# montyhall/bot7

Measured on AMD Instinct MI355X. Metric: EI candidates scored/sec at N=2048,d=32, higher is better.
Workload: dtype f64

## Files before the change

### bot7_amd/build.py

```python
import concurrent.futures
import os
import subprocess
import sys

HERE = os.path.dirname(os.path.abspath(__file__))
ROOT = os.path.dirname(HERE)
CSRC = os.path.join(HERE, "csrc")
BUILD = os.path.join(HERE, "_build")
OUT = os.path.join(HERE, "libbot7hip.so")
SOURCES = ["context.hip", "grid_api.hip", "gp_api.hip", "nominate.hip", "blr_api.hip", "sobol.hip", "covar.hip", "potrf.hip", "potrf_persist.hip", "posterior.hip", "score.hip", "extras.hip", "comm.hip", "group.hip", "blr_small.hip", "gp_small.hip", "kpost_small.hip", "batch.hip", "mes.hip"]
DIAG_ONLY_SOURCES = ["nll_small.hip"]
DIAG_OUT = os.path.join(ROOT, "tools", "_build", "libbot7hip_diag.so")
HEADERS = [os.path.join(CSRC, "b7_internal.h"), os.path.join(CSRC, "gemm_f64.h"), os.path.join(CSRC, "potrf_diag.h"), os.path.join(CSRC, "comm_rccl.h"), os.path.join(CSRC, "ksx_exp.h"), os.path.join(CSRC, "exp_table.h"), os.path.join(CSRC, "mes_math.h"),
           os.path.join(ROOT, "include", "bot7hip.h")]
HIPCC = os.environ.get("HIPCC", "/opt/rocm/bin/hipcc")
FLAGS = ["-O3", "-std=c++17", "-fPIC", "--offload-arch=gfx950", "-fno-fast-math", "-Wall",
         "-I" + os.path.join(ROOT, "include"), "-I" + CSRC, "-I/opt/rocm/include"]


def _stale(target, deps):
    if not os.path.exists(target):
        return True
    t = os.path.getmtime(target)
    return any(os.path.getmtime(d) > t for d in deps)


EXTRA_FLAGS = {"covar.hip": ["-mllvm", "-amdgpu-mfma-vgpr-form"], "batch.hip": ["-mllvm", "-amdgpu-mfma-vgpr-form"]}


def _compile(src, diag=False):
    obj = os.path.join(BUILD, ("diag_" if diag else "") + src.replace(".hip", ".o"))
    path = os.path.join(CSRC, src)
    if _stale(obj, [path] + HEADERS + [os.path.abspath(__file__)]):
        subprocess.check_call([HIPCC] + FLAGS + EXTRA_FLAGS.get(src, []) + (["-DB7_DIAG"] if diag else []) + ["-c", path, "-o", obj])
        return obj, True
    return obj, False


def _mentions_diag(src):
    return "B7_DIAG" in open(os.path.join(CSRC, src)).read()


def build_diag(verbose=False):
    build()
    os.makedirs(os.path.dirname(DIAG_OUT), exist_ok=True)
    todo = [s for s in SOURCES if _mentions_diag(s)] + DIAG_ONLY_SOURCES
    with concurrent.futures.ThreadPoolExecutor(max_workers=min(8, len(todo))) as ex:
        res = dict(zip(todo, ex.map(lambda s: _compile(s, True), todo)))
    objs = [res[s][0] if s in res else os.path.join(BUILD, s.replace(".hip", ".o")) for s in SOURCES + DIAG_ONLY_SOURCES]
    if any(ch for _, ch in res.values()) or _stale(DIAG_OUT, objs):
        subprocess.check_call([HIPCC, "-shared", "-fPIC", "--offload-arch=gfx950", "-o", DIAG_OUT] + objs +
                              ["-ldl", "-Wl,-rpath,/opt/rocm/lib", "-Wl,--no-undefined", "-Wl,-Bsymbolic"])
        if verbose:
            print("built", DIAG_OUT)
    return DIAG_OUT


def posterior_isa():
    out = os.path.join(BUILD, "posterior.s")
    path = os.path.join(CSRC, "posterior.hip")
    if _stale(out, [path] + HEADERS + [os.path.abspath(__file__)]):
        subprocess.check_call([HIPCC] + [f for f in FLAGS if f != "-fPIC"] + ["-S", "--cuda-device-only", "-Wno-unused-command-line-argument",
                                                                            path, "-o", out])
# ... 72 lines not shown
```

### bot7_amd/csrc/b7_internal.h

```cpp
#pragma once
#include <hip/hip_runtime.h>
#include <stddef.h>
#include <stdint.h>

#include <map>
#include <string>
#include <vector>

#include "bot7hip.h"

constexpr int B7_NPAD = 128;
constexpr int B7_PANEL = 64;
constexpr int B7_PERSIST_NMAX = 4096;
constexpr int B7_MROWS = 256;
constexpr int B7_MAX_D = 96;

constexpr int B7_TAB_VAL = 0;
constexpr int B7_TAB_IDX = 1;
constexpr int B7_TAB_STATUS = 2;
constexpr int B7_TAB_ROWS = 3;
constexpr int B7_TAB_ROW0 = 4;
constexpr int B7_TAB_W = B7_TAB_ROW0 + B7_MAX_D;
constexpr int B7_MAX_WORLD = 64;

// ... 89 lines not shown
  DevBuf w;
  DevBuf zsc;
  DevBuf zss;
  DevBuf K;
  DevBuf L;
  DevBuf Linv;
  DevBuf W;
  DevBuf dinv;
  DevBuf alpha;
  DevBuf resid;
  DevBuf atmp;
  DevBuf info;
  DevBuf ybuf;

  bool predicted = false;
  int64_t Mpred = 0;
  DevBuf mu;
  DevBuf var;
  DevBuf acc;
  bool acc_valid = false;
  int spin_us = 500;
  bool npad_small = true;
  bool potrf_small = true;
  bool blr_small = true;
  double fmin_scalar = 0.0;
  bool acc_fresh = false;
  int acc_kind = 0;
  DevBuf ks;
  size_t ks_bytes = (size_t)4 << 30;
  int diag_variant = 1;
  int inverse_inline = 1;
  PinnedBlock *pinned = nullptr, *pinned_dev = nullptr;
  std::vector<double> net_host;
  PinBuf pin_blr;
  PinBuf pin_eval;
  PinBuf pin_nll;
  bool fmin_staged = false;
  bool potrf_attrs_set = false;
  bool linv_done = false;
  int potrf_sched = 3;
  int syrk_small = 1;
  int potrf_defer = 1;
  int potrf_group = 2;
  struct JobList { DevBuf buf; int n = 0; };
  std::map<int, JobList> pjobs_cache;
  DevBuf pstamps;
  int pjobs_nb = 0, pjobs_n = 0;
  DevBuf bhyp, bw, bzsc, bzss, bK, bL, bdinv, bflags, binfo, bresid, bterms, bLinv, balpha, bmu, bvar;
  bool persist_attr_set = false, persist_stamps = false;
  int persist_helpers = 0;
  int persist_aborts = 0;
  int nll_small = 1;
  bool kpost_small = true;
  bool fit_small = true;
  int persist_fault = -1;
  int potrf_sched_saved = 0;
  DevBuf part;
  DevBuf ystar, mes_ticket;
  DevBuf mes_user;
  int mes_levels = 8;
  int mes_S = 0, mes_K = 0, mes_nb = 0;
  int64_t mes_M = 0;
  int mes_slot = 0;
  bool mes_valid = false;
  DevBuf ticket;
  DevBuf scratch;
  DevBuf tmpgrid;
  DevBuf tmpmu, tmpvar;
  DevBuf fant;
  DevBuf bel;
  DevBuf belvec;
  PinBuf pin_bel;
  DevBuf feat;
  size_t feat_zeroed_bytes = 0;
  int feat_z = -1;
  int64_t Mfeat = 0;
  int zdim = 0;
  uint64_t feat_version = 0, grid_version = 0;
  DevBuf netbuf;

  void *comm = nullptr;
  int comm_rank = 0, comm_world = 1;
  DevBuf slots;
  uint64_t *tab_host = nullptr;
  uint64_t *tab_host_dev = nullptr;
  struct b7_group *group = nullptr;
  bool group_busy = false;
  bool win_valid = false;
  int64_t win_idx1 = 0;
  int win_rank = -1, win_d = 0;
  double win_row[B7_MAX_D];
  int64_t shard_rows[B7_MAX_WORLD];
  int shard_world = 0;

  hipEvent_t tev[B7_MAX_TIMERS][2];
  bool tev_init = false;
  bool profile = false;
  std::map<std::string, PhaseStat> phases;
  struct PendingPhase { const char *name; hipEvent_t e0, e1; };
  std::vector<PendingPhase> pending;
  std::vector<hipEvent_t> free_events;
  hipEvent_t phase_e0 = nullptr;
};

int b7_fail(b7_ctx *c, int code, const char *fmt, ...);
#define B7_HIP(c, expr)                                                                          \
// ... 38 lines not shown
  int64_t s_w = 0, s_zsc = 0, s_zsh = 0, s_out = 0;
  const double *amp = nullptr;
  int64_t s_alpha = 0, s_mu = 0;
  const double *mean = nullptr;
};
struct ObsSet {
  const double *zsc;
  const double *zsh;
  int npad;
  const double *w = nullptr;
  KBatchDesc batch;
};
int launch_prep_obs_aux(b7_ctx *c, const double *xobs, const double *ls_dev, int N, int npad, double *zsc,
                        double *zsh);
int launch_k_generic(b7_ctx *c, const double *xq, int64_t rows, int64_t Mtotal, const ObsSet &o, double *out);
int launch_prep_obs(b7_ctx *c, const double *xobs, const double *lenscale_sq_dev, int N, int d);
int launch_kxx(b7_ctx *c, double diag_add);
int launch_ksx_batch(b7_ctx *c, int S, const double *xq, int64_t rows, int64_t Mtotal, const double *w, const double *zsc,
                     const double *zss, const double *amp_dev, const double *mean_dev, const double *alpha, double *ks,
                     int64_t s_out, double *mu, int64_t s_mu);
int launch_kxx_batch(b7_ctx *c, int B, const double *ls_dev, const double *amp_dev, const double *noise_dev, double *w,
                     double *zsc, double *zss, double *K);
int launch_ksx(b7_ctx *c, const double *xq, int64_t row0, int64_t rows, int64_t Mtotal, int d, double *ks,
               double *mu, int ycols);

struct FactorNote {
  bool alpha_done = false;
  int *report_written = nullptr;
};
int launch_potrf(b7_ctx *c, double extra, bool with_inverse, int *report_hint = nullptr, FactorNote *note = nullptr);
int launch_trtri(b7_ctx *c);
int launch_potrf_persist(b7_ctx *c, double extra, bool with_inverse);
int launch_nll_batch(b7_ctx *c, int B, const double *K, double *L, double *dinv, unsigned *flags, int *info,
                     const double *resid, double *terms);
int launch_nll_one(b7_ctx *c, const double *K, double *L, double *dinv, unsigned *flags, int *info, const double *resid,
                   double *terms, double extra);
size_t persist_flag_words_host(int nb);
int launch_potrf_small(b7_ctx *c, int B, const double *K, double *L, double *Linv, double *dinv, const double *resid, double *alpha,
                       double extra, int *info, int *report_dev, int64_t sK, int64_t sL, int64_t sdinv, int64_t svec, int sinfo);
int launch_blr_head_small(b7_ctx *c, const double *Z, int N, int z, int ldz, const double *yv, double alpha_prec, double beta,
                          int *report_dev);
int launch_blr_heads_small(b7_ctx *c, int S, const double *Z, int N, int z, int ldz, const double *yraw_dev, const double *hyp3_dev,
                           double *L, double *Linv, double *m, double *b, int *info, int *report_dev, double *terms);
int launch_post_heads(b7_ctx *c, int S, const double *Linv, const double *feat, int64_t rows, int64_t Mtotal, double *var, int64_t svar,
                      const double *zero_dev, const double *invbeta_dev);
int launch_gemv_rows_batch(b7_ctx *c, int S, const double *A, int lda, const double *x, int64_t sx, int n, const double *base_dev,
                           int64_t rows, double *y, int64_t sy);
int launch_nll_small(b7_ctx *c, int B, const double *hyp_dev, const double *hyp_host, double *terms_dev, int *info_dev,
                     unsigned *done_dev);
bool kpost_small_applies(const b7_ctx *c);
int launch_kpost_small(b7_ctx *c, int S, const double *xq, int64_t M, const double *w, const double *zsc, const double *zss,
                       const double *Linv, const double *alpha, const double *hyp_dev, double amp, double noise, double mean,
                       double *mu, double *var, int64_t sout);
bool gp_small_applies(const b7_ctx *c);
static inline bool fit_small_applies(const b7_ctx *c) {
  return c->fit_small && c->potrf_sched == 3 && c->inverse_inline && gp_small_applies(c);
}
int launch_nll_small8(b7_ctx *c, int B, const double *hyp_dev, const double *hyp_host, double *terms_dev, int *info_dev,
                      unsigned *done_dev);
int launch_fit_small(b7_ctx *c, int B, const double *hyp_dev, const double *hyp_host, double *hyp_out, double *w, double *zsc,
                     double *zss, double *L, double *Linv, double *dinv, double *alpha, double *resid, int *info_dev,
                     int *report_dev);
int launch_alpha(b7_ctx *c, int *report_dev = nullptr, int report_words = 0, const FactorNote &note = FactorNote());
int launch_alpha_batch(b7_ctx *c, int B, const double *Linv, const double *resid, double *alpha, const int *report_src = nullptr,
                       int *report_dev = nullptr, int report_words = 0);
int launch_fit_batch(b7_ctx *c, int B, const double *K, double *L, double *Linv, double *dinv, unsigned *flags, int *info);
int launch_nll_terms(b7_ctx *c, double *out_dev);
int launch_fro_norm_sq(b7_ctx *c, const double *A, int n, int ld, double *out_dev);
int launch_set_identity(b7_ctx *c);

int launch_post(b7_ctx *c, const double *ks, int64_t row0, int64_t rows, int64_t Mtotal, double *var);
int launch_post_batch(b7_ctx *c, int S, const double *Linv, const double *ks, int64_t sks, int64_t rows, int64_t Mtotal,
                      double *var, int64_t svar, const double *amp_dev, const double *noise_dev);

int launch_mean_multi(b7_ctx *c, const double *ks, int64_t row0, int64_t rows, int64_t Mtotal, double *mu);
int launch_gemm_nt(b7_ctx *c, const double *A, int lda, const double *B, int ldb, double *C, int ldc, int m, int n,
                   int k);
int launch_fantasy_cov(b7_ctx *c, const double *kpp, const double *g, double *S, int P, double diag_add);
int launch_fantasy_factor(b7_ctx *c, double *S, double *dinv_tmp, int *info_dev);
int launch_fantasy_sample(b7_ctx *c, const double *Lp, const double *mu, int P, int n, uint64_t seed, double *out);
int launch_add_diag(b7_ctx *c, double *S, int ld, int n, double v);

int launch_append_finalize(b7_ctx *c, const double *krow, const double *lvec, const double *uvec, const double *evec,
                           int *status_dev);
int launch_append_vectors(b7_ctx *c, const double *krow, double *lvec, double *uvec, double *part, double *evec);
int launch_mlp_forward(b7_ctx *c, const double *X, int64_t M, int d, const double *net_dev, const int *dims,
                       int n_layers, int activation, double *out, int ld_out);
int launch_mlp_forward_mean(b7_ctx *c, const double *X, int64_t M, int d, const double *net_dev, const int *dims,
                            int n_layers, int activation, double *out, int ld_out, const double *mvec, double mean0,
                            double *mu, bool *mean_done);
int launch_gemv_rows(b7_ctx *c, const double *A, int lda, const double *x, int n, double base, int64_t row0,
                     int64_t rows, int64_t Mtotal, double *y);
int launch_transpose_pad(b7_ctx *c, const double *Z, int n, int ldz, int z, double *Zt, int zpad, int nk);
int launch_blr_assemble(b7_ctx *c, const double *G, double *K, int z, int zpad, double alpha_prec, double beta);

int launch_score(b7_ctx *c, ScoreParams p, const double *mu, const double *var, int64_t M, int ycols, double *out, bool accumulate);
int launch_score_batch(b7_ctx *c, const ScoreParams &p, double *acc, int64_t M);
int launch_finish(b7_ctx *c, double *acc, int64_t M, double divisor, double *best_val, int64_t *best_idx1, bool logacc = false);
int launch_fill(b7_ctx *c, double *p, int64_t n, double v);
int launch_finish_slot(b7_ctx *c, double *acc, int64_t M, double divisor, uint64_t *tab_dev, int rank, int world,
                       int64_t offset, const double *grid, int d, bool all_slots, uint64_t *host_rec = nullptr,
                       unsigned *host_done = nullptr, bool logacc = false);

struct ExclRows {
  int n = 0;
  long long row[B7_BATCH_MAX];
// ... 105 lines not shown
```

### bot7_amd/csrc/context.hip

```cpp
#include <stdarg.h>
#include <stdio.h>
#include <stdlib.h>
#include <string.h>

#include "b7_internal.h"

static thread_local std::string g_create_err;

int b7_fail(b7_ctx *c, int code, const char *fmt, ...) {
  char buf[512];
  va_list ap;
  va_start(ap, fmt);
  vsnprintf(buf, sizeof(buf), fmt, ap);
  va_end(ap);
  if (c)
    c->err = buf;
  else
    g_create_err = buf;
  return code;
}

int b7_ensure(b7_ctx *c, DevBuf &b, size_t bytes) {
  if (bytes == 0) bytes = 16;
  if (b.cap >= bytes) return B7_OK;
// ... 73 lines not shown
int npad_of(const b7_ctx *c, int64_t n) { return (c->npad_small && n <= 64) ? 64 : (int)round_up(n, B7_NPAD); }

static int timers_init(b7_ctx *c) {
  if (c->tev_init) return B7_OK;
  for (int i = 0; i < B7_MAX_TIMERS; ++i) {
    B7_HIP(c, hipEventCreate(&c->tev[i][0]));
    B7_HIP(c, hipEventCreate(&c->tev[i][1]));
  }
  c->tev_init = true;
  return B7_OK;
}

extern "C" {

int b7_abi_version(void) { return B7_ABI_VERSION; }

int b7_create(b7_ctx **out, int device_id) {
  if (!out) return b7_fail(nullptr, B7_ERR_INVALID, "b7_create: out is NULL");
  *out = nullptr;
  int ndev = 0;
  hipError_t e = hipGetDeviceCount(&ndev);
  if (e != hipSuccess || ndev <= 0)
    return b7_fail(nullptr, B7_ERR_HIP, "no HIP device available (%s); libbot7hip has no CPU path",
                   e == hipSuccess ? "device count 0" : hipGetErrorString(e));
  if (device_id < 0 || device_id >= ndev)
    return b7_fail(nullptr, B7_ERR_INVALID, "device_id %d out of range [0,%d)", device_id, ndev);
  e = hipSetDevice(device_id);
  if (e != hipSuccess) return b7_fail(nullptr, B7_ERR_HIP, "hipSetDevice: %s", hipGetErrorString(e));
  hipDeviceProp_t prop;
  e = hipGetDeviceProperties(&prop, device_id);
  if (e != hipSuccess) return b7_fail(nullptr, B7_ERR_HIP, "hipGetDeviceProperties: %s", hipGetErrorString(e));
  if (strncmp(prop.gcnArchName, "gfx950", 6) != 0)
    return b7_fail(nullptr, B7_ERR_UNSUPPORTED, "device %d is %s; libbot7hip is built for gfx950 only", device_id,
                   prop.gcnArchName);
  b7_ctx *c = new b7_ctx();
  c->device = device_id;
  c->cus = prop.multiProcessorCount;
  b7_gp_default_opts(&c->opts);
  if (const char *pv = getenv("B7_SPIN_US")) c->spin_us = atoi(pv);
#ifdef B7_DIAG
  if (const char *pv = getenv("B7_DIAG_VARIANT")) c->diag_variant = atoi(pv);
  if (const char *pv = getenv("B7_NPAD_SMALL")) c->npad_small = atoi(pv) != 0;
  if (const char *pv = getenv("B7_POTRF_SMALL")) c->potrf_small = atoi(pv) != 0;
  if (getenv("B7_POTRF_SCHED") || getenv("B7_DIAG_VARIANT") || getenv("B7_INVERSE_INLINE")) c->potrf_small = c->fit_small = false;
  if (const char *pv = getenv("B7_BLR_SMALL")) c->blr_small = atoi(pv) != 0;
  if (const char *pv = getenv("B7_INVERSE_INLINE")) c->inverse_inline = atoi(pv);
  if (const char *pv = getenv("B7_POTRF_SCHED")) c->potrf_sched = atoi(pv);
  c->persist_stamps = getenv("B7_PERSIST_STAMPS") != nullptr;
  if (const char *pv = getenv("B7_PERSIST_HELPERS")) c->persist_helpers = atoi(pv);
  if (const char *pv = getenv("B7_PERSIST_FAULT")) c->persist_fault = atoi(pv);
  if (const char *pv = getenv("B7_NLL_SMALL")) c->nll_small = atoi(pv);
  if (const char *pv = getenv("B7_FIT_SMALL")) c->fit_small = atoi(pv) != 0;
  if (const char *pv = getenv("B7_KPOST_SMALL")) c->kpost_small = atoi(pv) != 0;
  if (const char *pv = getenv("B7_SYRK_SMALL")) c->syrk_small = atoi(pv) ? 1 : 0;
  if (const char *pv = getenv("B7_POTRF_DEFER")) c->potrf_defer = atoi(pv) ? 1 : 0;
  if (const char *pv = getenv("B7_POTRF_GROUP")) {
    const int g = atoi(pv);
    if (g >= 1 && g <= 8) c->potrf_group = g;
  }
#endif
  e = hipStreamCreateWithFlags(&c->stream, hipStreamNonBlocking);
  if (e == hipSuccess) e = hipEventCreateWithFlags(&c->ev_fit, hipEventDisableTiming);
  if (e == hipSuccess) e = hipHostMalloc((void **)&c->pinned, B7_PINNED_BYTES, hipHostMallocMapped);
  if (e == hipSuccess) e = hipHostGetDevicePointer((void **)&c->pinned_dev, c->pinned, 0);
  if (e != hipSuccess) {
    if (c->pinned) (void)hipHostFree(c->pinned);
    if (c->stream) (void)hipStreamDestroy(c->stream);
    delete c;
    return b7_fail(nullptr, B7_ERR_HIP, "stream / pinned result block creation: %s", hipGetErrorString(e));
  }
  if (b7_ensure(c, c->scratch, B7_SCRATCH_BYTES) != B7_OK) {
    g_create_err = c->err;
    b7_destroy(c);
    return B7_ERR_NOMEM;
  }
  *out = c;
  return B7_OK;
}

void b7_destroy(b7_ctx *c) {
  if (!c) return;
  (void)hipSetDevice(c->device);
  (void)hipStreamSynchronize(c->stream);
  (void)b7_comm_destroy(c);
  DevBuf *all[] = {&c->grid[0], &c->grid[1], &c->xobs, &c->w,     &c->zsc,  &c->zss,     &c->K,      &c->L,
                   &c->Linv,    &c->W,       &c->dinv, &c->alpha, &c->resid, &c->info,   &c->ybuf,   &c->mu,
                   &c->var,     &c->acc,     &c->ks,   &c->part,  &c->scratch, &c->tmpgrid, &c->tmpmu, &c->tmpvar, &c->fant, &c->feat, &c->netbuf, &c->atmp, &c->slots, &c->pstamps,
                   &c->bhyp, &c->bw, &c->bzsc, &c->bzss, &c->bK, &c->bL, &c->bdinv, &c->bflags, &c->binfo, &c->bresid, &c->bterms,
                   &c->bLinv, &c->balpha, &c->bmu, &c->bvar, &c->ticket, &c->bel, &c->belvec, &c->ystar, &c->mes_ticket, &c->mes_user};
  for (auto &kv : c->pjobs_cache) b7_release(kv.second.buf);
  for (DevBuf *b : all) b7_release(*b);
  if (c->tev_init)
    for (int i = 0; i < B7_MAX_TIMERS; ++i) {
      (void)hipEventDestroy(c->tev[i][0]);
      (void)hipEventDestroy(c->tev[i][1]);
    }
  resolve_phases(c);
  if (c->pinned) (void)hipHostFree(c->pinned);
  for (PinBuf *b : {&c->pin_eval, &c->pin_blr, &c->pin_nll, &c->pin_bel})
    if (b->host) (void)hipHostFree(b->host);
  if (c->tab_host) (void)hipHostFree(c->tab_host);
  for (hipEvent_t e : c->free_events) (void)hipEventDestroy(e);
  if (c->phase_e0) (void)hipEventDestroy(c->phase_e0);
  if (c->ev_fit) (void)hipEventDestroy(c->ev_fit);
  (void)hipStreamDestroy(c->stream);
  delete c;
// ... 72 lines not shown
```

### bot7_amd/csrc/gp_api.hip

```cpp
#include <math.h>
#include <string.h>

#include <chrono>

#include "b7_internal.h"

extern "C" __global__ void __launch_bounds__(256) resid_kernel(const double *__restrict__ y, double *__restrict__ r, int64_t nreal,
                                                               int64_t ntotal, double mean) {
  const int64_t e = (int64_t)blockIdx.x * blockDim.x + threadIdx.x;
  if (e < ntotal) r[e] = e < nreal ? y[e] - mean : 0.0;
}

extern "C" __global__ void __launch_bounds__(256) resid_batch_kernel(const double *__restrict__ y, double *__restrict__ r, int N,
                                                                     int Npad, const double *__restrict__ mean) {
  const int i = blockIdx.x * blockDim.x + threadIdx.x, b = blockIdx.y;
  if (i < Npad) r[(int64_t)b * Npad + i] = i < N ? y[i] - mean[b] : 0.0;
}

void launch_resid_batch(b7_ctx *c, int B, const double *mean_dev) {
  hipLaunchKernelGGL(resid_batch_kernel, dim3((c->Npad + 255) / 256, B), dim3(256), 0, c->stream, (const double *)c->ybuf.p,
                     (double *)c->bresid.p, c->N, c->Npad, mean_dev);
}

void persist_gave_up(b7_ctx *c) {
// ... 25 lines not shown
  int info = 1;
  double jitter = 0.0;
  {
    double *fro_dev = reinterpret_cast<double *>(reinterpret_cast<char *>(c->info.p) + 16);
    B7_TRY(launch_fro_norm_sq(c, (const double *)c->K.p, N, c->Npad, fro_dev));
    double fro = 0.0;
    B7_HIP(c, hipMemcpyAsync(&fro, fro_dev, sizeof(double), hipMemcpyDeviceToHost, c->stream));
    B7_HIP(c, hipStreamSynchronize(c->stream));
    const double max_eps = sqrt(fro);
    if (max_eps != max_eps)
      return b7_fail(c, B7_ERR_INVALID, "chol: the matrix contains NaN (check X_obs and the hyper-parameters)");
    double eps = c->opts.jitter_eps;
    for (;;) {
      if (eps > max_eps) {
        jitter = -1.0;
        B7_TRY(launch_set_identity(c));
        c->linv_done = false;
        if (note) *note = FactorNote();
        break;
      }
      eps = eps * c->opts.jitter_growth;
      B7_TRY(try_factor(c, eps, &info, with_inverse, note));
      if (info == 0) {
        jitter = eps;
        break;
      }
    }
  }
  *jitter_out = jitter;
  return B7_OK;
}

int chol_with_jitter(b7_ctx *c, double *jitter_out, int *info_first_out, bool with_inverse, FactorNote *note) {
  int info = 0;
  B7_TRY(try_factor(c, 0.0, &info, with_inverse, note));
  *info_first_out = info;
  *jitter_out = 0.0;
  if (info != 0) B7_TRY(jitter_retries(c, jitter_out, with_inverse, note));
  return B7_OK;
}

int64_t predict_chunk(const b7_ctx *c, int64_t M) {
  int64_t chunk = (int64_t)(c->ks_bytes / (sizeof(double) * (size_t)c->Npad)) / B7_MROWS * B7_MROWS;
  if (chunk < B7_MROWS) chunk = B7_MROWS;
  const int64_t Mpad = round_up(M, B7_MROWS);
  return chunk > Mpad ? Mpad : chunk;
}

int predict_into(b7_ctx *c, const double *xq, int64_t M, double *mu, double *var) {
  if (M == 0) return B7_OK;
  if (c->kpost_small && c->model_kind == 0 && kpost_small_applies(c))
    return launch_kpost_small(c, 1, xq, M, (const double *)c->w.p, (const double *)c->zsc.p, (const double *)c->zss.p,
                              (const double *)c->Linv.p, (const double *)c->alpha.p, nullptr, c->amp, c->noise, c->mean, mu, var, M);
  const int64_t chunk = predict_chunk(c, M), Mpad = round_up(M, B7_MROWS);
  B7_TRY(b7_ensure(c, c->ks, sizeof(double) * (size_t)chunk * c->Npad));
  for (int64_t row0 = 0; row0 < M; row0 += chunk) {
    int64_t rows = Mpad - row0 < chunk ? Mpad - row0 : chunk;
    B7_TRY(launch_ksx(c, xq, row0, rows, M, c->dfit, (double *)c->ks.p, mu, c->ycols));
    if (c->ycols > 1) B7_TRY(launch_mean_multi(c, (const double *)c->ks.p, row0, rows, M, mu));
    B7_TRY(launch_post(c, (const double *)c->ks.p, row0, rows, M, var));
  }
  return B7_OK;
}

int check_hyp(b7_ctx *c, const b7_hyp *hyp, int d) {
  if (!hyp || !hyp->lenscale_sq) return b7_fail(c, B7_ERR_INVALID, "gp_fit_hyp: NULL argument");
  for (int k = 0; k < d; ++k)
    if (!(hyp->lenscale_sq[k] > 0.0)) return b7_fail(c, B7_ERR_INVALID, "gp_fit: lenscale_sq[%d] must be > 0", k);
  if (!(hyp->amp > 0.0) || !(hyp->noise >= 0.0)) return b7_fail(c, B7_ERR_INVALID, "gp_fit: amp > 0, noise >= 0");
  return B7_OK;
}

int fit_front(b7_ctx *c, const b7_hyp *hyp, const double *ls_dev) {
  const int N = c->N, d = c->dfit, ycols = c->ycols;
  c->fitted = false;
  c->model_kind = 0;
  c->predicted = false;
  c->amp = hyp->amp;
  c->noise = hyp->noise;
  c->mean = hyp->mean;
  const int64_t ntotal = (int64_t)c->Npad * ycols;
  hipLaunchKernelGGL(resid_kernel, dim3((unsigned)((ntotal + 255) / 256)), dim3(256), 0, c->stream,
                     (const double *)c->ybuf.p, (double *)c->resid.p, (int64_t)N * ycols, ntotal, hyp->mean);
  B7_TRY(launch_prep_obs(c, (const double *)c->xobs.p, ls_dev, N, d));
  return launch_kxx(c, hyp->noise);
}

int fit_hyp_core(b7_ctx *c, const b7_hyp *hyp, double *nll_out, double *jitter_used, int *info_out,
                        bool then_predict) {
  if (!c) return B7_ERR_INVALID;
  if (!c->have_data) return b7_fail(c, B7_ERR_STATE, "gp_fit_hyp: call b7_gp_set_data first");
  const int N = c->N, d = c->dfit, ycols = c->ycols;
  B7_TRY(check_hyp(c, hyp, d));
  B7_HIP(c, hipSetDevice(c->device));

  double *ls_stage = c->pinned->vec, *ls_dev = b7_scratch(c)->lenscale;
  memcpy(ls_stage, hyp->lenscale_sq, sizeof(double) * d);
  const bool small = fit_small_applies(c);
  if (small) {
    ls_stage[d] = hyp->amp, ls_stage[d + 1] = hyp->noise, ls_stage[d + 2] = hyp->mean;
    c->fitted = false;
    c->model_kind = 0;
    c->predicted = false;
    c->amp = hyp->amp;
    c->noise = hyp->noise;
    c->mean = hyp->mean;
// ... 486 lines not shown
```

### bot7_amd/csrc/nominate.hip

```cpp
#include <string.h>

#include <algorithm>

#include "b7_internal.h"

int stage_fmin(b7_ctx *c, const double *fmin, double **fd_out) {
  if (c->ycols == 1) {
    c->fmin_scalar = fmin[0];
    *fd_out = nullptr;
    return B7_OK;
  }
  double *fh = c->pinned->fmin, *fd = b7_scratch(c)->fmin;
  if (!c->fmin_staged || memcmp(fh, fmin, sizeof(double) * c->ycols) != 0) {
    B7_HIP(c, hipStreamSynchronize(c->stream));
    memcpy(fh, fmin, sizeof(double) * c->ycols);
    c->fmin_staged = true;
  }
  B7_HIP(c, hipMemcpyAsync(fd, fh, sizeof(double) * c->ycols, hipMemcpyHostToDevice, c->stream));
  *fd_out = fd;
  return B7_OK;
}

ScoreParams score_params(const b7_ctx *c, const b7_score_spec *spec, const double *fd) {
  ScoreParams p;
// ... 39 lines not shown
  if (S < 1 || !hyps || !spec) return b7_fail(c, B7_ERR_INVALID, "eval_nominate: S >= 1, hyps and spec required");
  B7_TRY(nominate_args(c, "eval_nominate", spec, offset));
  if (!c->have_data) return b7_fail(c, B7_ERR_STATE, "eval_nominate: call b7_gp_set_data first");
  if (c->M > 0 && c->d != c->dfit)
    return b7_fail(c, B7_ERR_INVALID, "eval_nominate: grid dims %d != data dims %d", c->d, c->dfit);
  for (int s = 0; s < S; ++s) B7_TRY(check_hyp(c, &hyps[s], c->dfit));
  return mes_refuse(c, "eval_nominate", spec);
}

int pending_score(b7_ctx *c, int S, const b7_score_spec *spec, const double *fd, ScoreParams *out) {
  ScoreParams p = score_params(c, spec, fd);
  p.S = S, p.mu = (const double *)c->bmu.p, p.var = (const double *)c->bvar.p, p.stride = c->M;
  if (spec->kind == B7_SCORE_MES) B7_TRY(mes_search_for(c, &p, p.mu, p.var, p.stride, S, 0));
  *out = p;
  return B7_OK;
}

static int keep_slots_ensure(b7_ctx *c, int S) {
  const size_t n = (size_t)c->Npad;
  B7_TRY(b7_ensure(c, c->bw, sizeof(double) * (size_t)S * c->dpad));
  B7_TRY(b7_ensure(c, c->bzsc, sizeof(double) * (size_t)S * n * c->dpad));
  B7_TRY(b7_ensure(c, c->bzss, sizeof(double) * (size_t)S * n));
  return b7_ensure(c, c->bLinv, sizeof(double) * (size_t)S * n * n);
}
static int keep_sample(b7_ctx *c, BelKeep *keep, int S, int s) {
  if (!keep) return B7_OK;
  const size_t n = (size_t)c->Npad, mb = sizeof(double) * (size_t)c->M;
  B7_HIP(c, hipMemcpyAsync(keep->mu + (size_t)s * c->M, c->mu.p, mb, hipMemcpyDeviceToDevice, c->stream));
  B7_HIP(c, hipMemcpyAsync(keep->var + (size_t)s * c->M, c->var.p, mb, hipMemcpyDeviceToDevice, c->stream));
  if (S == 1) {
    keep->w = (const double *)c->w.p, keep->zsc = (const double *)c->zsc.p, keep->zss = (const double *)c->zss.p;
    keep->Linv = (const double *)c->Linv.p;
    return B7_OK;
  }
  keep->w = (const double *)c->bw.p, keep->zsc = (const double *)c->bzsc.p, keep->zss = (const double *)c->bzss.p;
  keep->Linv = (const double *)c->bLinv.p;
  if (c->w.p == (double *)c->bw.p + (size_t)s * c->dpad) return B7_OK;
  B7_HIP(c, hipMemcpyAsync((double *)c->bw.p + (size_t)s * c->dpad, c->w.p, sizeof(double) * c->dpad, hipMemcpyDeviceToDevice, c->stream));
  B7_HIP(c, hipMemcpyAsync((double *)c->bzsc.p + s * n * c->dpad, c->zsc.p, sizeof(double) * n * c->dpad, hipMemcpyDeviceToDevice, c->stream));
  B7_HIP(c, hipMemcpyAsync((double *)c->bzss.p + s * n, c->zss.p, sizeof(double) * n, hipMemcpyDeviceToDevice, c->stream));
  B7_HIP(c, hipMemcpyAsync((double *)c->bLinv.p + s * n * n, c->Linv.p, sizeof(double) * n * n, hipMemcpyDeviceToDevice, c->stream));
  return B7_OK;
}
static int keep_batch(b7_ctx *c, BelKeep *keep, int S) {
  if (!keep) return B7_OK;
  const size_t bytes = sizeof(double) * (size_t)S * c->M;
  B7_HIP(c, hipMemcpyAsync(keep->mu, c->bmu.p, bytes, hipMemcpyDeviceToDevice, c->stream));
  B7_HIP(c, hipMemcpyAsync(keep->var, c->bvar.p, bytes, hipMemcpyDeviceToDevice, c->stream));
  keep->w = (const double *)c->bw.p, keep->zsc = (const double *)c->bzsc.p, keep->zss = (const double *)c->bzss.p;
  keep->Linv = (const double *)c->bLinv.p;
  return B7_OK;
}

int eval_enqueue(b7_ctx *c, int S, const b7_hyp *hyps, const b7_score_spec *spec, ScoreParams *pend, BelKeep *keep) {
  const int d = c->dfit;
  B7_HIP(c, hipSetDevice(c->device));
  B7_TRY(b7_ensure(c, c->mu, sizeof(double) * (size_t)c->M * c->ycols));
  B7_TRY(b7_ensure(c, c->var, sizeof(double) * (size_t)c->M));
  B7_TRY(b7_ensure(c, c->acc, sizeof(double) * (size_t)c->M));
  B7_TRY(b7_ensure(c, c->ks, sizeof(double) * (size_t)predict_chunk(c, c->M) * c->Npad));
  if (spec->kind == B7_SCORE_MES) B7_TRY(mes_begin(c, S, c->M, c->mes_levels));
  const size_t hyp_doubles = (size_t)S * (d + 3), ls_bytes = sizeof(double) * hyp_doubles, rep_bytes = 16 * (size_t)S;
  B7_TRY(b7_pin_ensure(c, c->pin_eval, ls_bytes + rep_bytes, true));
  B7_TRY(b7_ensure(c, c->bhyp, ls_bytes));
  int *reports = static_cast<int *>(c->pin_eval.host);
  double *ls_host = reinterpret_cast<double *>(static_cast<char *>(c->pin_eval.host) + rep_bytes);
  const HypPack hp = hyp_pack(ls_host, S, d);
  for (int s = 0; s < S; ++s) {
    memcpy(hp.ls + (size_t)s * d, hyps[s].lenscale_sq, sizeof(double) * d);
    hp.amp[s] = hyps[s].amp;
    hp.noise[s] = hyps[s].noise;
    hp.mean[s] = hyps[s].mean;
  }
  memset(reports, 0xff, rep_bytes);
  const bool small = fit_small_applies(c);
  const bool batch = small || (S > 1 && c->ycols == 1 && c->potrf_sched == 3 && c->Npad <= B7_PERSIST_NMAX && c->inverse_inline);
  const int n = c->Npad;
  const size_t nn = (size_t)n * n;
  if (batch) {
    const size_t fw = persist_flag_words_host(n / B7_PANEL);
    B7_TRY(b7_ensure(c, c->bw, sizeof(double) * (size_t)S * c->dpad));
    B7_TRY(b7_ensure(c, c->bzsc, sizeof(double) * (size_t)S * n * c->dpad));
    B7_TRY(b7_ensure(c, c->bzss, sizeof(double) * (size_t)S * n));
    B7_TRY(b7_ensure(c, c->bLinv, sizeof(double) * S * nn));
    B7_TRY(b7_ensure(c, c->binfo, sizeof(int) * 4 * (size_t)S));
    B7_TRY(b7_ensure(c, c->balpha, sizeof(double) * (size_t)S * n));
    if (!small) {
      B7_TRY(b7_ensure(c, c->bK, sizeof(double) * S * nn));
      B7_TRY(b7_ensure(c, c->bL, sizeof(double) * S * nn));
      B7_TRY(b7_ensure(c, c->bdinv, sizeof(double) * (size_t)S * n * B7_PANEL));
      B7_TRY(b7_ensure(c, c->bflags, sizeof(unsigned) * S * fw));
      B7_TRY(b7_ensure(c, c->bresid, sizeof(double) * (size_t)S * n));
    }
  }
  if (!small) B7_HIP(c, hipMemcpyAsync(c->bhyp.p, ls_host, ls_bytes, hipMemcpyHostToDevice, c->stream));
  double *fd = nullptr;
  if (score_needs_fmin(spec->kind)) B7_TRY(stage_fmin(c, spec->fmin, &fd));

  acc_declare_zeros(c, spec->kind);
  if (batch) {
    const HypPack hd = hyp_pack(c->bhyp.p, S, d);
    const double *hyp_dev = hd.ls, *amp_dev = hd.amp, *noise_dev = hd.noise, *mean_dev = hd.mean;
    int *reports_dev = static_cast<int *>(c->pin_eval.dev);
    if (small) {
      const double *hyp_map = reinterpret_cast<const double *>(static_cast<const char *>(c->pin_eval.dev) + rep_bytes);
      B7_TRY(launch_fit_small(c, S, hyp_map, ls_host, (double *)c->bhyp.p, (double *)c->bw.p, (double *)c->bzsc.p, (double *)c->bzss.p,
                              nullptr, (double *)c->bLinv.p, nullptr, (double *)c->balpha.p, nullptr, (int *)c->binfo.p, reports_dev));
    } else {
      launch_resid_batch(c, S, mean_dev);
      B7_TRY(launch_kxx_batch(c, S, hyp_dev, amp_dev, noise_dev, (double *)c->bw.p, (double *)c->bzsc.p, (double *)c->bzss.p,
                              (double *)c->bK.p));
      if (n == 64 && c->potrf_small) {
        B7_TRY(launch_potrf_small(c, S, (const double *)c->bK.p, (double *)c->bL.p, (double *)c->bLinv.p, (double *)c->bdinv.p,
                                  (const double *)c->bresid.p, (double *)c->balpha.p, 0.0, (int *)c->binfo.p, reports_dev, (int64_t)nn,
                                  (int64_t)nn, (int64_t)n * B7_PANEL, (int64_t)n, 4));
      } else {
        B7_TRY(launch_fit_batch(c, S, (const double *)c->bK.p, (double *)c->bL.p, (double *)c->bLinv.p, (double *)c->bdinv.p,
                                (unsigned *)c->bflags.p, (int *)c->binfo.p));
        if (4 * S <= 256) {
          B7_TRY(launch_alpha_batch(c, S, (const double *)c->bLinv.p, (const double *)c->bresid.p, (double *)c->balpha.p,
                                    (const int *)c->binfo.p, reports_dev, 4 * S));
        } else {
          B7_TRY(launch_alpha_batch(c, S, (const double *)c->bLinv.p, (const double *)c->bresid.p, (double *)c->balpha.p));
          B7_HIP(c, hipMemcpyAsync(reports, c->binfo.p, rep_bytes, hipMemcpyDeviceToHost, c->stream));
        }
      }
    }
    const size_t row_bytes = sizeof(double) * (size_t)n;
    const int64_t Mpad = round_up(c->M, B7_MROWS);
    if (c->kpost_small && kpost_small_applies(c)) {
      B7_TRY(b7_ensure(c, c->bmu, sizeof(double) * (size_t)S * c->M));
      B7_TRY(b7_ensure(c, c->bvar, sizeof(double) * (size_t)S * c->M));
      B7_TRY(launch_kpost_small(c, S, (const double *)c->grid[c->grid_cur].p, c->M, (const double *)c->bw.p, (const double *)c->bzsc.p,
                                (const double *)c->bzss.p, (const double *)c->bLinv.p, (const double *)c->balpha.p, hyp_dev, 0.0, 0.0, 0.0,
                                (double *)c->bmu.p, (double *)c->bvar.p, c->M));
      B7_TRY(keep_batch(c, keep, S));
      B7_TRY(pending_score(c, S, spec, fd, pend));
      c->fitted = false;
      c->predicted = false;
    } else if ((size_t)Mpad * S * row_bytes <= c->ks_bytes) {
      B7_TRY(b7_ensure(c, c->ks, (size_t)Mpad * S * row_bytes));
      B7_TRY(b7_ensure(c, c->bmu, sizeof(double) * (size_t)S * c->M));
      B7_TRY(b7_ensure(c, c->bvar, sizeof(double) * (size_t)S * c->M));
      B7_TRY(launch_ksx_batch(c, S, (const double *)c->grid[c->grid_cur].p, Mpad, c->M, (const double *)c->bw.p,
                              (const double *)c->bzsc.p, (const double *)c->bzss.p, amp_dev, mean_dev,
                              (const double *)c->balpha.p, (double *)c->ks.p, (int64_t)Mpad * n, (double *)c->bmu.p, c->M));
      B7_TRY(launch_post_batch(c, S, (const double *)c->bLinv.p, (const double *)c->ks.p, (int64_t)Mpad * n, Mpad, c->M,
                               (double *)c->bvar.p, c->M, amp_dev, noise_dev));
      B7_TRY(keep_batch(c, keep, S));
      ScoreParams all;
      B7_TRY(pending_score(c, S, spec, fd, &all));
      B7_TRY(launch_score_batch(c, all, (double *)c->acc.p, c->M));
      c->fitted = false;
      c->predicted = false;
    } else {
      void *const zsc0 = c->zsc.p, *const zss0 = c->zss.p, *const w0 = c->w.p, *const alpha0 = c->alpha.p, *const linv0 = c->Linv.p;
      int rc = B7_OK;
      for (int s = 0; s < S && rc == B7_OK; ++s) {
        c->zsc.p = (double *)c->bzsc.p + (size_t)s * n * c->dpad;
        c->zss.p = (double *)c->bzss.p + (size_t)s * n;
        c->w.p = (double *)c->bw.p + (size_t)s * c->dpad;
        c->alpha.p = (double *)c->balpha.p + (size_t)s * n;
        c->Linv.p = (double *)c->bLinv.p + s * nn;
        c->amp = hyps[s].amp;
        c->noise = hyps[s].noise;
        c->mean = hyps[s].mean;
        c->model_kind = 0;
        c->fitted = true;
        rc = predict_into(c, (const double *)c->grid[c->grid_cur].p, c->M, (double *)c->mu.p, (double *)c->var.p);
        c->mes_slot = s;
        if (rc == B7_OK) rc = score_add(c, spec, fd);
        if (rc == B7_OK) rc = keep_sample(c, keep, S, s);
      }
      c->zsc.p = zsc0, c->zss.p = zss0, c->w.p = w0, c->alpha.p = alpha0, c->Linv.p = linv0;
      c->fitted = false;
      c->predicted = true;
      c->Mpred = c->M;
      B7_TRY(rc);
    }
  } else {
    if (keep && S > 1) B7_TRY(keep_slots_ensure(c, S));
    for (int s = 0; s < S; ++s) {
      B7_TRY(fit_front(c, &hyps[s], (const double *)c->bhyp.p + (size_t)s * d));
      int *report = static_cast<int *>(c->pin_eval.dev) + 4 * s;
      FactorNote note;
      B7_TRY(launch_potrf(c, 0.0, true, report, &note));
      if (!c->linv_done) B7_TRY(launch_trtri(c));
      B7_TRY(launch_alpha(c, report, 4, note));
      c->fitted = true;
      B7_TRY(predict_into(c, (const double *)c->grid[c->grid_cur].p, c->M, (double *)c->mu.p, (double *)c->var.p));
      c->predicted = true;
      c->Mpred = c->M;
      c->mes_slot = s;
      B7_TRY(score_add(c, spec, fd));
      B7_TRY(keep_sample(c, keep, S, s));
    }
    c->fitted = false;
  }
  return B7_OK;
}

bool reports_clean(b7_ctx *c, const int *reports, int S, bool persist) {
  bool clean = true, aborted = false;
  for (int s = 0; s < S; ++s) {
    clean = clean && reports[4 * s] == 0 && reports[4 * s + 1] == 0;
    aborted = aborted || reports[4 * s + 1] != 0;
  }
  if (aborted && persist) persist_gave_up(c);
  return clean;
}

int eval_redo(b7_ctx *c, int S, const b7_hyp *hyps, const b7_score_spec *spec, double *jitter_out, int *info_out, BelKeep *keep) {
  B7_HIP(c, hipSetDevice(c->device));
  if (keep && S > 1) B7_TRY(keep_slots_ensure(c, S));
  B7_TRY(acc_write_zeros(c));
  if (spec->kind == B7_SCORE_MES) B7_TRY(mes_begin(c, S, c->M, c->mes_levels));
  double *fd = nullptr;
  for (int s = 0; s < S; ++s) {
    B7_TRY(fit_hyp_core(c, &hyps[s], nullptr, jitter_out ? jitter_out + s : nullptr, info_out ? info_out + s : nullptr, true));
    c->predicted = true;
    c->Mpred = c->M;
    if (score_needs_fmin(spec->kind)) B7_TRY(stage_fmin(c, spec->fmin, &fd));
    c->mes_slot = s;
    B7_TRY(score_add(c, spec, fd));
    B7_TRY(keep_sample(c, keep, S, s));
  }
  return B7_OK;
}

static int score_ready(b7_ctx *c, const char *who) {
  if (!c->predicted || c->Mpred != c->M) return b7_fail(c, B7_ERR_STATE, "%s: call b7_gp_predict first", who);
  if (!c->acc_valid) return b7_fail(c, B7_ERR_STATE, "%s: call b7_score_reset first", who);
  return B7_OK;
}

static int upload_mv(b7_ctx *c, const double *mean, const double *var, int64_t M, int cc) {
  B7_TRY(b7_ensure(c, c->tmpmu, sizeof(double) * (size_t)M * cc));
  B7_TRY(b7_ensure(c, c->tmpvar, sizeof(double) * (size_t)M));
  B7_TRY(b7_ensure(c, c->tmpgrid, sizeof(double) * (size_t)M));
  B7_HIP(c, hipMemcpyAsync(c->tmpmu.p, mean, sizeof(double) * (size_t)M * cc, hipMemcpyHostToDevice, c->stream));
  B7_HIP(c, hipMemcpyAsync(c->tmpvar.p, var, sizeof(double) * (size_t)M, hipMemcpyHostToDevice, c->stream));
  return B7_OK;
}

static int score_compute(b7_ctx *c, const b7_score_spec &spec, const double *mean, const double *var, int64_t M, int cc, double *out) {
  if (M == 0) return B7_OK;
  B7_HIP(c, hipSetDevice(c->device));
  B7_TRY(upload_mv(c, mean, var, M, cc));
  double *fd = nullptr;
  if (score_needs_fmin(spec.kind)) {
    fd = b7_scratch(c)->fmin;
    B7_HIP(c, hipMemcpyAsync(fd, spec.fmin, sizeof(double) * cc, hipMemcpyHostToDevice, c->stream));
  }
  B7_TRY(launch_score(c, score_params(c, &spec, fd), (const double *)c->tmpmu.p, (const double *)c->tmpvar.p, M, cc,
                      (double *)c->tmpgrid.p, false));
  B7_HIP(c, hipMemcpyAsync(out, c->tmpgrid.p, sizeof(double) * (size_t)M, hipMemcpyDeviceToHost, c->stream));
  B7_HIP(c, hipStreamSynchronize(c->stream));
  return B7_OK;
}

extern "C" {

int b7_eval_nominate(b7_ctx *c, int S, const b7_hyp *hyps, const b7_score_spec *spec, int64_t global_row_offset,
                     double *best_val, int64_t *best_idx1, double *jitter_out, int *info_out) {
  if (!c) return B7_ERR_INVALID;
// ... 99 lines not shown
```

Baseline: 16.14 million.

## Add fused mid-size kernel computing cross-covariance, mean and variance without materialising Ks

Adds a kpost_mid kernel for 128<N<=512 that computes the cross-covariance tiles on the fly with MFMA, multiplies them by Linv streamed through double-buffered LDS, and reduces the mean and variance in one pass. It replaces the separate ksx_batch and post_batch launches and drops the global Ks buffer, cutting memory traffic and launch count. Belief-keeping paths hold it off. The cost is that Linv tiles are re-streamed for every group of query rows, and the kernel uses large LDS and many registers, which may limit occupancy.

```diff
diff --git a/bot7_amd/build.py b/bot7_amd/build.py
--- a/bot7_amd/build.py
+++ b/bot7_amd/build.py
@@ -8,7 +8,7 @@
 CSRC = os.path.join(HERE, "csrc")
 BUILD = os.path.join(HERE, "_build")
 OUT = os.path.join(HERE, "libbot7hip.so")
-SOURCES = ["context.hip", "grid_api.hip", "gp_api.hip", "nominate.hip", "blr_api.hip", "sobol.hip", "covar.hip", "potrf.hip", "potrf_persist.hip", "posterior.hip", "score.hip", "extras.hip", "comm.hip", "group.hip", "blr_small.hip", "gp_small.hip", "kpost_small.hip", "batch.hip", "mes.hip"]
+SOURCES = ["context.hip", "grid_api.hip", "gp_api.hip", "nominate.hip", "blr_api.hip", "sobol.hip", "covar.hip", "potrf.hip", "potrf_persist.hip", "posterior.hip", "score.hip", "extras.hip", "comm.hip", "group.hip", "blr_small.hip", "gp_small.hip", "kpost_small.hip", "kpost_mid.hip", "batch.hip", "mes.hip"]
 DIAG_ONLY_SOURCES = ["nll_small.hip"]
 DIAG_OUT = os.path.join(ROOT, "tools", "_build", "libbot7hip_diag.so")
 HEADERS = [os.path.join(CSRC, "b7_internal.h"), os.path.join(CSRC, "gemm_f64.h"), os.path.join(CSRC, "potrf_diag.h"), os.path.join(CSRC, "comm_rccl.h"), os.path.join(CSRC, "ksx_exp.h"), os.path.join(CSRC, "exp_table.h"), os.path.join(CSRC, "mes_math.h"),
diff --git a/bot7_amd/csrc/b7_internal.h b/bot7_amd/csrc/b7_internal.h
--- a/bot7_amd/csrc/b7_internal.h
+++ b/bot7_amd/csrc/b7_internal.h
@@ -165,6 +165,8 @@
   int persist_aborts = 0;
   int nll_small = 1;
   bool kpost_small = true;
+  bool kpost_mid = true;
+  bool kpost_mid_hold = false;
   bool fit_small = true;
   int persist_fault = -1;
   int potrf_sched_saved = 0;
@@ -309,6 +311,10 @@
 int launch_kpost_small(b7_ctx *c, int S, const double *xq, int64_t M, const double *w, const double *zsc, const double *zss,
                        const double *Linv, const double *alpha, const double *hyp_dev, double amp, double noise, double mean,
                        double *mu, double *var, int64_t sout);
+bool kpost_mid_applies(const b7_ctx *c);
+int launch_kpost_mid(b7_ctx *c, int S, const double *xq, int64_t M, const double *w, const double *zsc, const double *zss,
+                     const double *Linv, const double *alpha, const double *hyp_dev, double amp, double noise, double mean,
+                     double *mu, double *var, int64_t sout);
 bool gp_small_applies(const b7_ctx *c);
 static inline bool fit_small_applies(const b7_ctx *c) {
   return c->fit_small && c->potrf_sched == 3 && c->inverse_inline && gp_small_applies(c);
diff --git a/bot7_amd/csrc/context.hip b/bot7_amd/csrc/context.hip
--- a/bot7_amd/csrc/context.hip
+++ b/bot7_amd/csrc/context.hip
@@ -149,6 +149,7 @@
   if (const char *pv = getenv("B7_NLL_SMALL")) c->nll_small = atoi(pv);
   if (const char *pv = getenv("B7_FIT_SMALL")) c->fit_small = atoi(pv) != 0;
   if (const char *pv = getenv("B7_KPOST_SMALL")) c->kpost_small = atoi(pv) != 0;
+  if (const char *pv = getenv("B7_KPOST_MID")) c->kpost_mid = atoi(pv) != 0;
   if (const char *pv = getenv("B7_SYRK_SMALL")) c->syrk_small = atoi(pv) ? 1 : 0;
   if (const char *pv = getenv("B7_POTRF_DEFER")) c->potrf_defer = atoi(pv) ? 1 : 0;
   if (const char *pv = getenv("B7_POTRF_GROUP")) {
diff --git a/bot7_amd/csrc/gp_api.hip b/bot7_amd/csrc/gp_api.hip
--- a/bot7_amd/csrc/gp_api.hip
+++ b/bot7_amd/csrc/gp_api.hip
@@ -101,6 +101,9 @@
   if (c->kpost_small && c->model_kind == 0 && kpost_small_applies(c))
     return launch_kpost_small(c, 1, xq, M, (const double *)c->w.p, (const double *)c->zsc.p, (const double *)c->zss.p,
                               (const double *)c->Linv.p, (const double *)c->alpha.p, nullptr, c->amp, c->noise, c->mean, mu, var, M);
+  if (c->kpost_mid && !c->kpost_mid_hold && c->model_kind == 0 && kpost_mid_applies(c))
+    return launch_kpost_mid(c, 1, xq, M, (const double *)c->w.p, (const double *)c->zsc.p, (const double *)c->zss.p,
+                            (const double *)c->Linv.p, (const double *)c->alpha.p, nullptr, c->amp, c->noise, c->mean, mu, var, M);
   const int64_t chunk = predict_chunk(c, M), Mpad = round_up(M, B7_MROWS);
   B7_TRY(b7_ensure(c, c->ks, sizeof(double) * (size_t)chunk * c->Npad));
   for (int64_t row0 = 0; row0 < M; row0 += chunk) {
diff --git a/bot7_amd/csrc/kpost_mid.hip b/bot7_amd/csrc/kpost_mid.hip
--- /dev/null
+++ b/bot7_amd/csrc/kpost_mid.hip
@@ -0,0 +1,233 @@
+#include "b7_internal.h"
+#include "gemm_f64.h"
+#include "ksx_exp.h"
+
+namespace {
+
+__constant__ double exp2_tab_km[128];
+
+constexpr int KM_THREADS = 512;
+constexpr int KM_SLAB = 8 * 4 * 64;
+
+struct KmArgs {
+  const double *xq;
+  int64_t M;
+  int d, N, npad, S;
+  const double *w, *zsc, *zss, *Linv, *alpha;
+  const double *hyp;
+  double amp, noise, mean;
+  double *mu, *var;
+  int64_t sout;
+  int var_with_noise, clamp;
+  double var_min;
+};
+
+template <int DPAD>
+__host__ __device__ constexpr int km_stage_doubles() { return KM_SLAB + 16 * DPAD; }
+template <int DPAD>
+__host__ __device__ constexpr int km_lds_doubles(int npad) { return 2 * km_stage_doubles<DPAD>() + 2 * npad + DPAD + 128; }
+
+struct KmCursor {
+  int t, jb, J;
+  __device__ __forceinline__ void advance(int NT, int ntile) {
+    const int rows = NT - 8 * t < 8 ? NT - 8 * t : 8;
+    if (++J < (jb < t ? 8 : rows)) return;
+    J = 0;
+    if (++jb <= t) return;
+    jb = 0;
+    if (++t == ntile) t = 0;
+  }
+};
+
+template <int DPAD, int KERN>
+__global__ void __launch_bounds__(KM_THREADS) kpost_mid_kernel(KmArgs a) {
+  constexpr int KS = DPAD / 4, STG = km_stage_doubles<DPAD>();
+  extern __shared__ __align__(16) double sm[];
+  const int tid = threadIdx.x, lane = tid & 63, wave = __builtin_amdgcn_readfirstlane(tid >> 6), lr = lane & 15, lq = lane >> 4;
+  const int s = blockIdx.y, npad = a.npad, d = a.d;
+  const int NT = (a.N + 15) >> 4, ntile = (NT + 7) >> 3;
+  double *zs = sm + 2 * STG, *al = zs + npad, *wv = al + npad, *tab = wv + DPAD;
+  const double amp = a.hyp ? a.hyp[(size_t)a.S * d + s] : a.amp;
+  const double noise = a.hyp ? a.hyp[(size_t)a.S * (d + 1) + s] : a.noise;
+  const double meanc = a.hyp ? a.hyp[(size_t)a.S * (d + 2) + s] : a.mean;
+  const double *Li = a.Linv + (size_t)s * npad * npad, *zc = a.zsc + (size_t)s * npad * DPAD;
+  for (int e = tid; e < 16 * NT; e += KM_THREADS) {
+    zs[e] = a.zss[(size_t)s * npad + e];
+    al[e] = a.alpha[(size_t)s * npad + e];
+  }
+  if (tid < DPAD) wv[tid] = a.w[(size_t)s * DPAD + tid];
+  if (tid < 128) tab[tid] = amp * exp2_tab_km[tid];
+  const int srow = tid >> 2, sq = tid & 3, sI = srow >> 4;
+  const int sdst = (sI * 4 + sq) * 64 + (srow & 15);
+  const int zdst = KM_SLAB + ((tid % DPAD) >> 2) * 64 + (tid & 3) * 16 + tid / DPAD;
+  d4_t gl = {0.0, 0.0, 0.0, 0.0};
+  double gz = 0.0;
+  auto fetch = [&](const KmCursor &q) {
+    const int rows = NT - 8 * q.t < 8 ? NT - 8 * q.t : 8, lo = q.jb == q.t ? q.J : 0;
+    if (sI >= lo && sI < rows)
+      gl = *reinterpret_cast<const d4_t *>(Li + (size_t)(128 * q.t + srow) * npad + 128 * q.jb + 16 * q.J + 4 * sq);
+    if (tid < 16 * DPAD) gz = zc[(size_t)(16 * (8 * q.jb + q.J)) * DPAD + tid];
+  };
+  auto stash = [&](double *b) {
+#pragma unroll
+    for (int g = 0; g < 4; ++g) b[sdst + 16 * g] = gl[g];
+    if (tid < 16 * DPAD) b[zdst] = gz;
+  };
+  KmCursor nxt{0, 0, 0};
+  fetch(nxt);
+  nxt.advance(NT, ntile);
+  stash(sm);
+  __syncthreads();
+  int par = 0;
+  const double var_add = a.var_with_noise ? noise : 0.0;
+  double *mu = a.mu + (size_t)s * a.sout, *var = a.var + (size_t)s * a.sout;
+  const int64_t nstrips = (a.M + 15) >> 4, ngroups = (nstrips + 7) >> 3;
+  for (int64_t grp = blockIdx.x; grp < ngroups; grp += gridDim.x) {
+    const int64_t st = grp * 8 + wave;
+    double xf[KS], hq;
+    {
+      int64_t g = st * 16 + lr;
+      g = g < a.M ? g : a.M - 1;
+      const double *px = a.xq + g * d;
+      double sx = 0.0;
+#pragma unroll
+      for (int k = 0; k < DPAD; ++k) {
+        const double v = k < d ? px[k] : 0.0;
+        sx += (v * v) * wv[k];
+        if ((k & 3) == lq) xf[k >> 2] = v;
+      }
+      hq = 0.5 * sx;
+    }
+    double mac[4] = {0.0, 0.0, 0.0, 0.0};
+    double colss[2] = {0.0, 0.0};
+    for (int t = 0; t < ntile; ++t) {
+      const int rows = NT - 8 * t < 8 ? NT - 8 * t : 8;
+      d4_t acc[8];
+#pragma unroll
+      for (int I = 0; I < 8; ++I) acc[I] = d4_t{0.0, 0.0, 0.0, 0.0};
+      for (int jb = 0; jb <= t; ++jb) {
+        const int nj = jb < t ? 8 : rows;
+        for (int J = 0; J < nj; ++J) {
+          const double *cur = sm + par * STG;
+          const int lo = jb == t ? J : 0, js = 8 * jb + J;
+          fetch(nxt);
+          nxt.advance(NT, ntile);
+          double af[8][4];
+#pragma unroll
+          for (int I = 0; I < 8; ++I)
+#pragma unroll
+            for (int q = 0; q < 4; ++q) af[I][q] = cur[(I * 4 + q) * 64 + lane];
+          d4_t c = {0.0, 0.0, 0.0, 0.0};
+#pragma unroll
+          for (int k4 = 0; k4 < KS; ++k4) c = mfma_f64(cur[KM_SLAB + k4 * 64 + lane], xf[k4], c);
+          double arg[4], kv[4];
+#pragma unroll
+          for (int r = 0; r < 4; ++r) arg[r] = (c[r] - hq) - zs[16 * js + lq + 4 * r];
+          cov_nonpos4<KERN>(arg, tab, kv);
+          asm volatile("" : "+v"(kv[0]), "+v"(kv[1]), "+v"(kv[2]), "+v"(kv[3]));
+          if (t == ntile - 1) {
+#pragma unroll
+            for (int r = 0; r < 4; ++r) mac[r] = __builtin_fma(kv[r], al[16 * js + lq + 4 * r], mac[r]);
+          }
+#pragma unroll
+          for (int I = 0; I < 8; ++I) {
+            if (I >= lo && I < rows) {
+#pragma unroll
+              for (int q = 0; q < 4; ++q) acc[I] = mfma_f64(af[I][q], kv[q], acc[I]);
+            }
+          }
+          stash(sm + (par ^ 1) * STG);
+          __syncthreads();
+          par ^= 1;
+        }
+      }
+#pragma unroll
+      for (int h = 0; h < 2; ++h) {
+        double sh = 0.0;
+#pragma unroll
+        for (int I = 4 * h; I < 4 * h + 4; ++I)
+#pragma unroll
+          for (int r = 0; r < 4; ++r) sh = __builtin_fma(acc[I][r], acc[I][r], sh);
+        colss[h] += sh;
+      }
+    }
+    double v[4];
+#pragma unroll
+    for (int r = 0; r < 4; ++r) {
+      v[r] = mac[r];
+      v[r] += __shfl_xor(v[r], 16);
+      v[r] += __shfl_xor(v[r], 32);
+    }
+    const double msum = (v[0] + v[1]) + (v[2] + v[3]);
+    double v0 = colss[0], v1 = colss[1];
+    v0 += __shfl_xor(v0, 16);
+    v0 += __shfl_xor(v0, 32);
+    v1 += __shfl_xor(v1, 16);
+    v1 += __shfl_xor(v1, 32);
+    const int64_t g = st * 16 + lr;
+    if (lane < 16 && g < a.M) {
+      mu[g] = meanc + msum;
+      double sq2 = v0;
+      sq2 += v1;
+      double o = (amp + -1.0 * sq2) + var_add;
+      if (a.clamp) o = (o < a.var_min) ? a.var_min : o;
+      var[g] = o;
+    }
+  }
+}
+
+int ensure_km_table(b7_ctx *c) {
+  static bool done[64] = {false};
+  if (c->device < 64 && done[c->device]) return B7_OK;
+  B7_HIP(c, hipMemcpyToSymbol(HIP_SYMBOL(exp2_tab_km), b7_exp2_tab, sizeof(b7_exp2_tab)));
+  if (c->device < 64) done[c->device] = true;
+  return B7_OK;
+}
+
+template <int DPAD, int KERN>
+int km_launch(b7_ctx *c, const KmArgs &a) {
+  B7_TRY(ensure_km_table(c));
+  const size_t lds = sizeof(double) * (size_t)km_lds_doubles<DPAD>(512);
+  static bool attr_done[64] = {false};
+  if (c->device >= 64 || !attr_done[c->device]) {
+    B7_HIP(c, hipFuncSetAttribute(reinterpret_cast<const void *>(kpost_mid_kernel<DPAD, KERN>), hipFuncAttributeMaxDynamicSharedMemorySize,
+                                  (int)lds));
+    if (c->device < 64) attr_done[c->device] = true;
+  }
+  const int64_t ngroups = (a.M + 127) / 128;
+  int64_t gx = c->cus / a.S;
+  if (gx > ngroups) gx = ngroups;
+  if (gx < 1) gx = 1;
+  hipLaunchKernelGGL((kpost_mid_kernel<DPAD, KERN>), dim3((unsigned)gx, (unsigned)a.S), dim3(KM_THREADS), lds, c->stream, a);
+  B7_HIP(c, hipGetLastError());
+  return B7_OK;
+}
+
+template <int DPAD>
+int km_dispatch(b7_ctx *c, const KmArgs &a) {
+  return c->kernel == B7_KERNEL_MATERN52 ? km_launch<DPAD, B7_KERNEL_MATERN52>(c, a) : km_launch<DPAD, B7_KERNEL_ARDSE>(c, a);
+}
+
+}
+
+bool kpost_mid_applies(const b7_ctx *c) { return c->Npad > 128 && c->Npad <= 512 && c->N > 128 && c->dfit <= 32 && c->ycols == 1; }
+
+int launch_kpost_mid(b7_ctx *c, int S, const double *xq, int64_t M, const double *w, const double *zsc, const double *zss,
+                     const double *Linv, const double *alpha, const double *hyp_dev, double amp, double noise, double mean,
+                     double *mu, double *var, int64_t sout) {
+  PhaseScope ps(c, "kpost");
+  if (M <= 0) return B7_OK;
+  KmArgs a = {};
+  a.xq = xq, a.M = M, a.d = c->dfit, a.N = c->N, a.npad = c->Npad, a.S = S;
+  a.w = w, a.zsc = zsc, a.zss = zss, a.Linv = Linv, a.alpha = alpha, a.hyp = hyp_dev;
+  a.amp = amp, a.noise = noise, a.mean = mean;
+  a.mu = mu, a.var = var, a.sout = sout;
+  a.var_with_noise = c->opts.var_with_noise, a.clamp = c->opts.var_clamp, a.var_min = c->opts.var_min;
+  switch (c->dpad) {
+    case 4: return km_dispatch<4>(c, a);
+    case 8: return km_dispatch<8>(c, a);
+    case 16: return km_dispatch<16>(c, a);
+    case 32: return km_dispatch<32>(c, a);
+    default: return b7_fail(c, B7_ERR_UNSUPPORTED, "kpost_mid: dpad %d", c->dpad);
+  }
+}
diff --git a/bot7_amd/csrc/nominate.hip b/bot7_amd/csrc/nominate.hip
--- a/bot7_amd/csrc/nominate.hip
+++ b/bot7_amd/csrc/nominate.hip
@@ -115,8 +115,16 @@
   return B7_OK;
 }
 
+struct KpostMidHold {
+  b7_ctx *c;
+  bool was;
+  KpostMidHold(b7_ctx *c, bool hold) : c(c), was(c->kpost_mid_hold) { c->kpost_mid_hold = was || hold; }
+  ~KpostMidHold() { c->kpost_mid_hold = was; }
+};
+
 int eval_enqueue(b7_ctx *c, int S, const b7_hyp *hyps, const b7_score_spec *spec, ScoreParams *pend, BelKeep *keep) {
   const int d = c->dfit;
+  const KpostMidHold hold(c, keep != nullptr);
   B7_HIP(c, hipSetDevice(c->device));
   B7_TRY(b7_ensure(c, c->mu, sizeof(double) * (size_t)c->M * c->ycols));
   B7_TRY(b7_ensure(c, c->var, sizeof(double) * (size_t)c->M));
@@ -202,14 +210,21 @@
       c->fitted = false;
       c->predicted = false;
     } else if ((size_t)Mpad * S * row_bytes <= c->ks_bytes) {
-      B7_TRY(b7_ensure(c, c->ks, (size_t)Mpad * S * row_bytes));
       B7_TRY(b7_ensure(c, c->bmu, sizeof(double) * (size_t)S * c->M));
       B7_TRY(b7_ensure(c, c->bvar, sizeof(double) * (size_t)S * c->M));
-      B7_TRY(launch_ksx_batch(c, S, (const double *)c->grid[c->grid_cur].p, Mpad, c->M, (const double *)c->bw.p,
-                              (const double *)c->bzsc.p, (const double *)c->bzss.p, amp_dev, mean_dev,
-                              (const double *)c->balpha.p, (double *)c->ks.p, (int64_t)Mpad * n, (double *)c->bmu.p, c->M));
-      B7_TRY(launch_post_batch(c, S, (const double *)c->bLinv.p, (const double *)c->ks.p, (int64_t)Mpad * n, Mpad, c->M,
-                               (double *)c->bvar.p, c->M, amp_dev, noise_dev));
+      const bool mid = c->kpost_mid && !c->kpost_mid_hold && kpost_mid_applies(c);
+      if (mid) {
+        B7_TRY(launch_kpost_mid(c, S, (const double *)c->grid[c->grid_cur].p, c->M, (const double *)c->bw.p, (const double *)c->bzsc.p,
+                                (const double *)c->bzss.p, (const double *)c->bLinv.p, (const double *)c->balpha.p, hyp_dev, 0.0, 0.0, 0.0,
+                                (double *)c->bmu.p, (double *)c->bvar.p, c->M));
+      } else {
+        B7_TRY(b7_ensure(c, c->ks, (size_t)Mpad * S * row_bytes));
+        B7_TRY(launch_ksx_batch(c, S, (const double *)c->grid[c->grid_cur].p, Mpad, c->M, (const double *)c->bw.p,
+                                (const double *)c->bzsc.p, (const double *)c->bzss.p, amp_dev, mean_dev,
+                                (const double *)c->balpha.p, (double *)c->ks.p, (int64_t)Mpad * n, (double *)c->bmu.p, c->M));
+        B7_TRY(launch_post_batch(c, S, (const double *)c->bLinv.p, (const double *)c->ks.p, (int64_t)Mpad * n, Mpad, c->M,
+                                 (double *)c->bvar.p, c->M, amp_dev, noise_dev));
+      }
       B7_TRY(keep_batch(c, keep, S));
       ScoreParams all;
       B7_TRY(pending_score(c, S, spec, fd, &all));
@@ -274,6 +289,7 @@
 }
 
 int eval_redo(b7_ctx *c, int S, const b7_hyp *hyps, const b7_score_spec *spec, double *jitter_out, int *info_out, BelKeep *keep) {
+  const KpostMidHold hold(c, keep != nullptr);
   B7_HIP(c, hipSetDevice(c->device));
   if (keep && S > 1) B7_TRY(keep_slots_ensure(c, S));
   B7_TRY(acc_write_zeros(c));
```

Result: no change. 16.16 million, median of 6 (+0.1%).
